# vghuy17ck1/svt-av1-psyex

Hardware: AMD Instinct MI355X
Metric: ME+RD-cost Mpixels/s (2160p10 preset-6) (higher is better)
Workload: dtype u8 SAD / i32 transforms; 1 GPU; 3840x2160 10-bit synthetic pan sequence, preset 6 (M6) search controls at qp 35; step = 16 pictures (4 current pictures x ref distance 1,2,4,8; R=2): open-loop ME of all 2040 b64 + full-pel pred + RD chain (64x64,32x32,16x16 DCT_DCT, 10-bit, b quantizer; qcoeff + recon + scalars written); 3 picture sets alternate from step to step

## Files before the change

### svt-av1-psyex_amd/csrc/rd_kernel.hip

```cpp
#include <hip/hip_runtime.h>
#include <math.h>
#include <stdint.h>
#include <string.h>
#include <type_traits>
#include "svt_hip_internal.h"
#include "../../include/svt_hip_dsp.h"

#include "txfm_core.h"

namespace {

struct RdParams {
    SvtHipRdBatchDesc d;
    const int16_t    *iscan[3];
    int               tx_size;
};

template <typename T> __device__ __forceinline__ int ldpix(const void *p, size_t i) { return (int)static_cast<const T *>(p)[i]; }

template <int LW> __device__ __forceinline__ u64 seg_sum_u64(u64 v) {
#pragma unroll
    for (int o = LW / 2; o > 0; o >>= 1) v += __shfl_xor(v, o, 64);
    return v;
}
template <int LW> __device__ __forceinline__ uint32_t seg_sum_u32(uint32_t v) {
#pragma unroll
    for (int o = LW / 2; o > 0; o >>= 1) v += __shfl_xor(v, o, 64);
    return v;
}
template <int LW> __device__ __forceinline__ uint32_t seg_max_u32(uint32_t v) {
#pragma unroll
    for (int o = LW / 2; o > 0; o >>= 1) { const uint32_t t = __shfl_xor(v, o, 64); v = t > v ? t : v; }
    return v;
}

__host__ __device__ constexpr int rd_lanes_per_block(int ts) { return tx_wide(ts) > tx_high(ts) ? tx_wide(ts) : tx_high(ts); }
__host__ __device__ constexpr int rd_blocks_per_wave(int ts) { return 64 / rd_lanes_per_block(ts); }

#ifndef SVT_RD_WAVES_64
#define SVT_RD_WAVES_64 2
#endif
#ifndef SVT_RD_WAVES_32
#define SVT_RD_WAVES_32 4
#endif
#ifndef SVT_RD_RESIDUAL_AHEAD
#define SVT_RD_RESIDUAL_AHEAD 8
#endif
#ifndef SVT_RD_SCAN_AHEAD
#define SVT_RD_SCAN_AHEAD 16
#endif
#ifndef SVT_RD_WAVES_16
#define SVT_RD_WAVES_16 4
#endif
__host__ __device__ constexpr int rd_waves_per_simd(int ts) {
    return rd_lanes_per_block(ts) == 64 ? SVT_RD_WAVES_64 : rd_lanes_per_block(ts) == 32 ? SVT_RD_WAVES_32 : SVT_RD_WAVES_16;
}
template <int TS, int BD> __global__ void __launch_bounds__(64, rd_waves_per_simd(TS)) rd_tx_kernel(const RdParams p) {
    constexpr int W = tx_wide(TS), H = tx_high(TS), WP = W > 32 ? 32 : W, HP = H > 32 ? 32 : H, NP = WP * HP;
    constexpr int LW = rd_lanes_per_block(TS), BPW = rd_blocks_per_wave(TS);
    constexpr bool kShift32 = LW != 32;
    constexpr int PA = W + 1, PB = WP + 1;
    constexpr int ROW_CLAMP = BD == 8 ? 16 : 18, COL_CLAMP = 16;
    constexpr bool RECT = (W == 2 * H || H == 2 * W);
    using Pix = typename std::conditional<BD == 8, uint8_t, uint16_t>::type;
    __shared__ int32_t lds[BPW][H * PA];
    const int      lane = threadIdx.x, blk = lane / LW, l = lane % LW;
    const uint32_t job   = blockIdx.x * BPW + blk;
    const bool     valid = job < p.d.n_jobs;
    int32_t *A = lds[blk];
    const SvtHipTxJob jb = p.d.jobs[valid ? job : 0];
    const int tt = jb.tx_type & 15, vt = c_vtx[tt], ht = c_htx[tt];
    const bool ud = (vt == 2), lr = (ht == 2);
    const Pix *src  = static_cast<const Pix *>(p.d.src) + jb.src_offset;
    const Pix *pred = static_cast<const Pix *>(p.d.pred) + jb.pred_offset;
    const int8_t *fsh = c_fwd_shift[TS];
    const int bit_col = c_fwd_cos_col[ilog2c(W) - 2][ilog2c(H) - 2], bit_row = c_fwd_cos_row[ilog2c(W) - 2][ilog2c(H) - 2];

    constexpr int RUN = W < 8 ? W : 8, RPR = W / RUN;
    typedef Pix __attribute__((ext_vector_type(RUN), aligned(sizeof(Pix)))) RunU;
    uint32_t rmax = 0;
    {
        HiLo rhl;
        constexpr int NIT = (RPR * H + LW - 1) / LW, kResidualAhead = NIT < SVT_RD_RESIDUAL_AHEAD ? NIT : SVT_RD_RESIDUAL_AHEAD;
        for (int it0 = 0; it0 < NIT; it0 += kResidualAhead) {
            RunU sv[kResidualAhead], pv[kResidualAhead];
#pragma unroll
            for (int j = 0; j < kResidualAhead; j++) {
                const int i = l + (it0 + j) * LW;
                if (it0 + j < NIT && i < RPR * H) {
                    const int r = i / RPR, c = (i - r * RPR) * RUN;
                    sv[j] = *reinterpret_cast<const RunU *>(src + (size_t)r * p.d.src_stride + c);
                    pv[j] = *reinterpret_cast<const RunU *>(pred + (size_t)r * p.d.pred_stride + c);
                }
            }
#pragma unroll
            for (int j = 0; j < kResidualAhead; j++) {
                const int i = l + (it0 + j) * LW;
                if (it0 + j < NIT && i < RPR * H) {
                    const int r = i / RPR, c = (i - r * RPR) * RUN;
#pragma unroll
                    for (int k = 0; k < RUN; k++) {
                        const int32_t d = (int16_t)((int16_t)sv[j][k] - (int16_t)pv[j][k]);
                        A[r * PA + c + k] = d;
                        rhl.take(d);
                    }
                }
            }
        }
        rmax = rhl.max_abs();
    }
    const bool fast_col = pass_fits_17_bits((uint32_t)__builtin_amdgcn_readfirstlane((int)seg_max_u32<64>(rmax)) << (fsh[0] > 0 ? fsh[0] : 0), H);
    __syncthreads();
    uint32_t cmax = 0;
    if (l < W) {
        int32_t x[H];
#pragma unroll
        for (int r = 0; r < H; r++) x[r] = A[(ud ? H - 1 - r : r) * PA + l];
        shift_vec<H>(x, fsh[0]);
        if (fast_col) { fwd_1d<H, 2>(x, vt, bit_col); shift_vec<H, kShift32>(x, fsh[1]); } else { fwd_1d<H, 0>(x, vt, bit_col); shift_vec<H>(x, fsh[1]); }
        const int oc = lr ? W - 1 - l : l;
#pragma unroll
        for (int r = 0; r < H; r++) A[r * PA + oc] = x[r];
        cmax = vec_max_abs<H>(x);
    }
    const bool fast_row = pass_fits_17_bits((uint32_t)__builtin_amdgcn_readfirstlane((int)seg_max_u32<64>(cmax)), W);
    __syncthreads();
    uint32_t comax = 0;
    if (l < H) {
        int32_t x[W];
#pragma unroll
        for (int c = 0; c < W; c++) x[c] = A[l * PA + c];
        if (fast_row) { fwd_1d<W, 2>(x, ht, bit_row); shift_vec<W, kShift32>(x, fsh[2]); } else { fwd_1d<W, 0>(x, ht, bit_row); shift_vec<W>(x, fsh[2]); }
        if constexpr (RECT) {
#pragma unroll
            for (int c = 0; c < W; c++) x[c] = rshift64((i64)x[c] * 5793, 12);
        }
#pragma unroll
        for (int c = 0; c < W; c++) A[l * PA + c] = x[c];
        comax = vec_max_abs<W>(x);
    }
    const bool q24 = (uint32_t)__builtin_amdgcn_readfirstlane((int)seg_max_u32<64>(comax)) < (1u << 16);
    __syncthreads();
    const int pf = jb.pf_shape & 3;
    const int keep_w = pf == 3 ? 1 : (W >> pf), keep_h = pf == 3 ? 1 : (H >> pf);
    u64 tq = 0;
    if (pf == 0) if constexpr (W > 32 || H > 32) {
        for (int i = l; i < W * H; i += LW) {
            const int r = i / W, c = i - r * W;
            if (r >= HP || c >= WP) { const int32_t v = A[r * PA + c]; tq += (u64)((i64)v * v); }
        }
        tq = seg_sum_u64<LW>(tq);
    }
    if constexpr (W > 32 || H > 32) __syncthreads();
    const SvtHipQuantRow q = p.d.quant_rows[jb.quant_row];
    const int     log_scale = p.d.quant_kind == 2 ? 0 : c_log_scale[TS];
    const int16_t *iscan    = p.iscan[(tt >= 10) ? ((tt & 1) ? 2 : 1) : 0];
    const uint8_t *qm = (tt < 9) ? p.d.qmatrix : nullptr, *iqm = (tt < 9) ? p.d.iqmatrix : nullptr;
    uint32_t satd = 0, eob = 0, qsum = 0;
    int32_t  dc_q = 0;
    u64      dres = 0, dpred = 0;
    int32_t *co_out = (p.d.coeff && valid) ? p.d.coeff + (size_t)job * NP : nullptr;
    int32_t *q_out  = (p.d.qcoeff && valid) ? p.d.qcoeff + (size_t)job * NP : nullptr;
    int32_t *dq_out = (p.d.dqcoeff && valid) ? p.d.dqcoeff + (size_t)job * NP : nullptr;
    const int32_t zb_c[2]  = {log_scale ? ((q.zbin[0] + (1 << (log_scale - 1))) >> log_scale) : q.zbin[0], log_scale ? ((q.zbin[1] + (1 << (log_scale - 1))) >> log_scale) : q.zbin[1]};
    const int32_t rnd_c[2] = {log_scale ? ((q.round[0] + (1 << (log_scale - 1))) >> log_scale) : q.round[0], log_scale ? ((q.round[1] + (1 << (log_scale - 1))) >> log_scale) : q.round[1]};
    const bool fast_q = q24 && !qm && p.d.quant_kind == 0 && !co_out && !dq_out && __all(pf == 0);
    if (fast_q) {
        static_assert(NP % LW == 0, "every lane of a block walks the same number of coefficients");
        constexpr int kScanAhead = NP / LW < SVT_RD_SCAN_AHEAD ? ((NP / LW) & ~1) : SVT_RD_SCAN_AHEAD;
        static_assert(kScanAhead >= 2 && kScanAhead % 2 == 0 && NP / LW >= kScanAhead, "ahead of the loop");
        uint32_t scan2[kScanAhead / 2];
#pragma unroll
        for (int k = 0; k < kScanAhead; k += 2) scan2[k / 2] = (uint32_t)(uint16_t)iscan[l + LW * k] | ((uint32_t)(uint16_t)iscan[l + LW * (k + 1)] << 16);
        auto one = [&](int rc, int32_t zb, int32_t rnd, int32_t quant, int32_t qshift, int32_t deq, int ahead = -1) {
            const int r = rc / WP, c = rc - r * WP;
            const int32_t co = A[r * PA + c], sign = co >> 31, a = (co ^ sign) - sign;
            satd += (uint32_t)a;
            int32_t t = a + rnd;
            if (BD == 8) t = t > 32767 ? 32767 : t;
            const int32_t tmp = mul24_shr(t, quant, 11) + (t << 5);
            int32_t qv = mul24_shr(tmp, qshift, 21 - log_scale);
            qv = a >= zb ? qv : 0;
            const int32_t dq = __mul24(qv, deq) >> log_scale;
            const int32_t qs = (qv ^ sign) - sign, dqs = (dq ^ sign) - sign;
            uint32_t e;
            if (ahead >= 0) e = qv ? ((scan2[ahead >> 1] >> (16 * (ahead & 1))) & 0xFFFFu) + 1u : 0u;
            else e = qv ? (uint32_t)iscan[rc] + 1u : 0u;
            eob = e > eob ? e : eob;
            qsum += (uint32_t)(qv > 63 ? 63 : qv);
            const int32_t dd = a - dq;
            dres += (u64)(uint32_t)__mul24(dd, dd);
            dpred += (u64)(uint32_t)__umul24((uint32_t)a, (uint32_t)a);
            A[r * PB + c] = dqs;
            if (q_out) q_out[rc] = qs;
            return qs;
        };
        const int ac0 = l != 0;
        dc_q = one(l, zb_c[ac0], rnd_c[ac0], q.quant[ac0], q.quant_shift[ac0], q.dequant[ac0], 0);
        const int32_t zb1 = zb_c[1], rnd1 = rnd_c[1], quant1 = q.quant[1], qshift1 = q.quant_shift[1], deq1 = q.dequant[1];
#pragma unroll
        for (int k = 1; k < kScanAhead; k++) one(l + LW * k, zb1, rnd1, quant1, qshift1, deq1, k);
        if constexpr (LW >= 32) {
            static_assert((NP / LW - kScanAhead) % 2 == 0, "pairs");
            for (int rc = l + kScanAhead * LW; rc < NP; rc += 2 * LW) {
                one(rc, zb1, rnd1, quant1, qshift1, deq1);
                one(rc + LW, zb1, rnd1, quant1, qshift1, deq1);
            }
        } else {
#pragma unroll 4
            for (int rc = l + kScanAhead * LW; rc < NP; rc += LW) one(rc, zb1, rnd1, quant1, qshift1, deq1);
        }
    } else
    for (int rc = l; rc < NP; rc += LW) {
        const int r = rc / WP, c = rc - r * WP, ac = rc != 0;
        const bool kept = pf == 0 || (c < keep_w && r < keep_h);
        const int32_t co = kept ? A[r * PA + c] : 0, sign = co < 0 ? -1 : 0, a = (co ^ sign) - sign;
        satd += (uint32_t)a;
        int32_t qv = 0, dq = 0;
        const int32_t wt = qm ? qm[rc] : 32, iwt = qm ? iqm[rc] : 32;
        if (q24 && !qm) {
            if (p.d.quant_kind == 0) {
                if (a >= zb_c[ac]) {
                    int32_t t = a + rnd_c[ac];
                    if (BD == 8) t = t > 32767 ? 32767 : t;
                    const int32_t tmp = mul24_shr(t, q.quant[ac], 11) + (t << 5);
                    qv = mul24_shr(tmp, q.quant_shift[ac], 21 - log_scale);
                    dq = __mul24(qv, (int32_t)q.dequant[ac]) >> log_scale;
                }
            } else {
                const bool keep = (a << (1 + log_scale)) >= q.dequant[ac];
                if (keep) {
                    int32_t t = a + (log_scale ? ((q.round_fp[ac] + (1 << (log_scale - 1))) >> log_scale) : q.round_fp[ac]);
                    if (BD == 8) t = t < -32768 ? -32768 : (t > 32767 ? 32767 : t);
                    qv = mul24_shr(t, q.quant_fp[ac], 16 - log_scale);
                    dq = __mul24(qv, (int32_t)q.dequant[ac]) >> log_scale;
                }
            }
        } else if (p.d.quant_kind == 0 && !qm) {
            const int32_t zb = zb_c[ac];
            if (a >= zb) {
                int32_t t = a + rnd_c[ac];
                if (BD == 8) t = t > 32767 ? 32767 : t;
                const int32_t tw  = t << 5;
                const int32_t tmp = (int32_t)(((i64)tw * q.quant[ac]) >> 16) + tw;
                qv = (int32_t)(((i64)tmp * q.quant_shift[ac]) >> (16 - log_scale + 5));
                dq = (qv * (int32_t)q.dequant[ac]) >> log_scale;
            }
        } else if (p.d.quant_kind == 0) {
            const int32_t zb = log_scale ? ((q.zbin[ac] + (1 << (log_scale - 1))) >> log_scale) : q.zbin[ac];
            if ((i64)a * wt >= ((i64)zb << 5)) {
                i64 t = (i64)a + (log_scale ? ((q.round[ac] + (1 << (log_scale - 1))) >> log_scale) : q.round[ac]);
                if (BD == 8) t = t < -32768 ? -32768 : (t > 32767 ? 32767 : t);
                t *= wt;
                qv = (int32_t)(((((t * q.quant[ac]) >> 16) + t) * q.quant_shift[ac]) >> (16 - log_scale + 5));
                const int32_t deq = ((int32_t)q.dequant[ac] * iwt + 16) >> 5;
                dq = (qv * deq) >> log_scale;
            }
        } else if (!qm) {
            const bool keep = (BD == 8) ? (((i64)a << (1 + log_scale)) >= (int32_t)q.dequant[ac]) : ((a << (1 + log_scale)) >= q.dequant[ac]);
            if (keep) {
                i64 t = (i64)a + (log_scale ? ((q.round_fp[ac] + (1 << (log_scale - 1))) >> log_scale) : q.round_fp[ac]);
                if (BD == 8) t = t < -32768 ? -32768 : (t > 32767 ? 32767 : t);
                qv = (int32_t)((t * q.quant_fp[ac]) >> (16 - log_scale));
                dq = (qv * (int32_t)q.dequant[ac]) >> log_scale;
            }
        } else {
            if ((i64)a * wt >= ((int32_t)q.dequant[ac] << (5 - (1 + log_scale)))) {
                i64 t = (i64)a + (log_scale ? ((q.round_fp[ac] + (1 << (log_scale - 1))) >> log_scale) : q.round_fp[ac]);
                if (BD == 8) t = t < -32768 ? -32768 : (t > 32767 ? 32767 : t);
                qv = (int32_t)((t * q.quant_fp[ac] * wt) >> (16 - log_scale + 5));
                const int32_t deq = ((int32_t)q.dequant[ac] * iwt + 16) >> 5;
                dq = (qv * deq) >> log_scale;
            }
        }
        const int32_t qs = (qv ^ sign) - sign, dqs = (dq ^ sign) - sign;
        if (qv) { const uint32_t e = (uint32_t)iscan[rc] + 1; eob = e > eob ? e : eob; }
        qsum += (uint32_t)(qv > 63 ? 63 : qv);
        if (rc == 0) dc_q = qs;
        const i64 dd = (i64)co - dqs;
        dres += (u64)(dd * dd);
        dpred += (u64)((i64)co * co);
        A[r * PB + c] = dqs;
        if (co_out) co_out[rc] = co;
        if (q_out) q_out[rc] = qs;
        if (dq_out) dq_out[rc] = dqs;
    }
    satd  = seg_sum_u32<LW>(satd);
    qsum  = seg_sum_u32<LW>(qsum);
    eob   = seg_max_u32<LW>(eob);
    dres  = seg_sum_u64<LW>(dres);
    dpred = seg_sum_u64<LW>(dpred);
    __syncthreads();
    int32_t xr[W];
    uint32_t irmax = 0;
    if (l < H) {
#pragma unroll
        for (int c = 0; c < W; c++) {
            int32_t v = (l < HP && c < WP) ? A[l * PB + c] : 0;
            if constexpr (RECT) v = rshift64((i64)v * 2896, 12);
            xr[c] = clampv(v, BD + 8);
        }
        irmax = vec_max_abs<W>(xr);
    }
    const bool fast_irow = ipass_fits_18_bits((uint32_t)__builtin_amdgcn_readfirstlane((int)seg_max_u32<64>(irmax)), W);
    uint32_t icmax = 0;
    if (l < H) {
        if (fast_irow) inv_1d<W, ROW_CLAMP, 2>(xr, ht); else inv_1d<W, ROW_CLAMP, 1>(xr, ht);
        shift_vec<W, kShift32>(xr, c_inv_shift0[TS]);
#pragma unroll
        for (int c = 0; c < W; c++) A[l * PA + c] = xr[c];
        icmax = vec_max_abs<W>(xr);
    }
    const bool fast_icol = ipass_fits_18_bits((uint32_t)__builtin_amdgcn_readfirstlane((int)seg_max_u32<64>(icmax)), H);
    __syncthreads();
    u64 sse = 0;
    if (l < W) {
        int32_t x[H];
        const int ic = lr ? W - 1 - l : l;
#pragma unroll
        for (int r = 0; r < H; r++) x[r] = (r < HP) ? clampv(A[r * PA + ic], BD + 6 > 16 ? BD + 6 : 16) : 0;
        if (fast_icol) inv_1d<H, COL_CLAMP, 2>(x, vt); else inv_1d<H, COL_CLAMP, 1>(x, vt);
        shift_vec<H, kShift32>(x, -4);
#pragma unroll
        for (int r = 0; r < H; r++) A[r * PA + l] = x[ud ? H - 1 - r : r];
    }
    __syncthreads();
    {
        Pix *rec = (p.d.recon && valid) ? static_cast<Pix *>(p.d.recon) + jb.pred_offset : nullptr;
        constexpr int NIT = (RPR * H + LW - 1) / LW;
        RunU pv[NIT], sv[NIT];
#pragma unroll
        for (int it = 0; it < NIT; it++) {
            const int i = l + it * LW;
            if (i < RPR * H) {
                const int r = i / RPR, c = (i - r * RPR) * RUN;
                pv[it] = *reinterpret_cast<const RunU *>(pred + (size_t)r * p.d.pred_stride + c);
                sv[it] = *reinterpret_cast<const RunU *>(src + (size_t)r * p.d.src_stride + c);
            }
        }
#pragma unroll
        for (int it = 0; it < NIT; it++) {
            const int i = l + it * LW;
            if (i < RPR * H) {
                const int r = i / RPR, c = (i - r * RPR) * RUN;
                RunU out;
#pragma unroll
                for (int k = 0; k < RUN; k++) {
                    int v = (int)pv[it][k] + A[r * PA + c + k];
                    v = v < 0 ? 0 : (v > (1 << BD) - 1 ? (1 << BD) - 1 : v);
                    out[k] = (Pix)v;
                    const int e = (int)sv[it][k] - v;
                    sse += (u64)((uint32_t)e * (uint32_t)e);
                }
                if (rec) *reinterpret_cast<RunU *>(rec + (size_t)r * p.d.pred_stride + c) = out;
            }
        }
    }
    sse = seg_sum_u64<LW>(sse);
    if (l == 0 && valid) {
        p.d.eob[job]  = (uint16_t)eob;
        p.d.satd[job] = satd;
        p.d.dist_coeff[2 * (size_t)job]     = dres;
        p.d.dist_coeff[2 * (size_t)job + 1] = dpred;
        p.d.three_quad_energy[job] = tq;
        p.d.sse[job]  = sse;
        if (p.d.cul_level) p.d.cul_level[job] = (uint8_t)((qsum > 63 ? 63 : qsum) | (dc_q < 0 ? 64 : 0)) + (uint8_t)(dc_q > 0 ? 128 : 0);
    }
}

struct InvParams {
    SvtHipInvTxBatchDesc d;
};
template <int TS, int BD, typename Pix> __global__ void __launch_bounds__(64, rd_waves_per_simd(TS)) inv_tx_kernel(const InvParams p) {
    constexpr int W = tx_wide(TS), H = tx_high(TS), WP = W > 32 ? 32 : W, HP = H > 32 ? 32 : H, NP = WP * HP;
    constexpr int LW = rd_lanes_per_block(TS), BPW = rd_blocks_per_wave(TS);
    constexpr bool kShift32 = LW != 32;
    constexpr int PA = W + 1, PB = WP + 1;
    constexpr int ROW_CLAMP = BD == 8 ? 16 : 18, COL_CLAMP = 16;
    constexpr bool RECT = (W == 2 * H || H == 2 * W);
    __shared__ int32_t lds[BPW][H * PA];
    const int      lane = threadIdx.x, blk = lane / LW, l = lane % LW;
    const uint32_t job   = blockIdx.x * BPW + blk;
    const bool     valid = job < p.d.n_jobs;
    int32_t *A = lds[blk];
    const SvtHipTxJob jb = p.d.jobs[valid ? job : 0];
    const int tt = jb.tx_type & 15, vt = c_vtx[tt], ht = c_htx[tt];
    const bool ud = (vt == 2), lr = (ht == 2);
    const Pix *pred = static_cast<const Pix *>(p.d.pred) + jb.pred_offset;
    const int32_t *dq = p.d.dqcoeff + (size_t)(valid ? job : 0) * NP;
    for (int rc = l; rc < NP; rc += LW) { const int r = rc / WP, c = rc - r * WP; A[r * PB + c] = dq[rc]; }
    __syncthreads();
    int32_t xr[W];
    uint32_t irmax = 0;
    if (l < H) {
#pragma unroll
        for (int c = 0; c < W; c++) {
            int32_t v = (l < HP && c < WP) ? A[l * PB + c] : 0;
            if constexpr (RECT) v = rshift64((i64)v * 2896, 12);
            xr[c] = clampv(v, BD + 8);
        }
        irmax = vec_max_abs<W>(xr);
    }
    const bool fast_irow = ipass_fits_18_bits((uint32_t)__builtin_amdgcn_readfirstlane((int)seg_max_u32<64>(irmax)), W);
    uint32_t icmax = 0;
    if (l < H) {
        if (fast_irow) inv_1d<W, ROW_CLAMP, 2>(xr, ht); else inv_1d<W, ROW_CLAMP, 1>(xr, ht);
        shift_vec<W, kShift32>(xr, c_inv_shift0[TS]);
#pragma unroll
        for (int c = 0; c < W; c++) A[l * PA + c] = xr[c];
        icmax = vec_max_abs<W>(xr);
    }
    const bool fast_icol = ipass_fits_18_bits((uint32_t)__builtin_amdgcn_readfirstlane((int)seg_max_u32<64>(icmax)), H);
    __syncthreads();
    if (l < W) {
        int32_t x[H];
        const int ic = lr ? W - 1 - l : l;
#pragma unroll
        for (int r = 0; r < H; r++) x[r] = (r < HP) ? clampv(A[r * PA + ic], BD + 6 > 16 ? BD + 6 : 16) : 0;
        if (fast_icol) inv_1d<H, COL_CLAMP, 2>(x, vt); else inv_1d<H, COL_CLAMP, 1>(x, vt);
        shift_vec<H, kShift32>(x, -4);
#pragma unroll
        for (int r = 0; r < H; r++) A[r * PA + l] = x[ud ? H - 1 - r : r];
    }
    __syncthreads();
    if (valid) {
        Pix *rec = static_cast<Pix *>(p.d.recon) + jb.src_offset;
        for (int i = l; i < W * H; i += LW) {
            const int r = i / W, c = i - r * W;
            int v = (int)pred[(size_t)r * p.d.pred_stride + c] + A[r * PA + c];
            v = v < 0 ? 0 : (v > (1 << BD) - 1 ? (1 << BD) - 1 : v);
            rec[(size_t)r * p.d.recon_stride + c] = (Pix)v;
        }
    }
}

template <int BD, typename Pix> int launch_inv(SvtHipContext *ctx, const InvParams &p) {
    const dim3 b(64);
#define CASE(S) case S: hipLaunchKernelGGL((inv_tx_kernel<S, BD, Pix>), dim3((p.d.n_jobs + rd_blocks_per_wave(S) - 1) / rd_blocks_per_wave(S)), b, 0, ctx->stream, p); break;
    switch (p.d.tx_size) {
        CASE(0) CASE(1) CASE(2) CASE(3) CASE(4) CASE(5) CASE(6) CASE(7) CASE(8) CASE(9) CASE(10) CASE(11) CASE(12) CASE(13) CASE(14) CASE(15) CASE(16) CASE(17) CASE(18)
    default: return svt_hip_fail(ctx, SVT_HIP_ERR_BAD_PARAM, "tx_size %d", p.d.tx_size);
    }
#undef CASE
    SVT_HIP_CHECK(ctx, hipGetLastError());
    return SVT_HIP_OK;
}

struct FwdParams {
    SvtHipFwdTxBatchDesc d;
};
template <int TS> __global__ void __launch_bounds__(64, rd_waves_per_simd(TS)) fwd_tx_kernel(const FwdParams p) {
    constexpr int W = tx_wide(TS), H = tx_high(TS);
    constexpr int LW = rd_lanes_per_block(TS), BPW = rd_blocks_per_wave(TS);
    constexpr int PA = W + 1;
    constexpr bool RECT = (W == 2 * H || H == 2 * W);
    __shared__ int32_t lds[BPW][H * PA];
    const int      lane = threadIdx.x, blk = lane / LW, l = lane % LW;
    const uint32_t job   = blockIdx.x * BPW + blk;
    const bool     valid = job < p.d.n_jobs;
    int32_t *A = lds[blk];
    const SvtHipTxJob jb = p.d.jobs[valid ? job : 0];
    const int tt = jb.tx_type & 15, vt = c_vtx[tt], ht = c_htx[tt];
    const bool ud = (vt == 2), lr = (ht == 2);
    const int16_t *res = p.d.residual + jb.src_offset;
    const int8_t *fsh = c_fwd_shift[TS];
    const int bit_col = c_fwd_cos_col[ilog2c(W) - 2][ilog2c(H) - 2], bit_row = c_fwd_cos_row[ilog2c(W) - 2][ilog2c(H) - 2];
    uint32_t rmax = 0;
    for (int i = l; i < W * H; i += LW) {
        const int r = i / W, c = i - r * W;
        const int32_t d = res[(size_t)r * p.d.residual_stride + c];
        A[r * PA + c] = d;
        rmax = max(rmax, (uint32_t)(d < 0 ? -d : d));
    }
    const bool fast_col = pass_fits_17_bits((uint32_t)__builtin_amdgcn_readfirstlane((int)seg_max_u32<64>(rmax)) << (fsh[0] > 0 ? fsh[0] : 0), H);
    __syncthreads();
    uint32_t cmax = 0;
    if (l < W) {
        int32_t x[H];
#pragma unroll
        for (int r = 0; r < H; r++) x[r] = A[(ud ? H - 1 - r : r) * PA + l];
        shift_vec<H>(x, fsh[0]);
        if (fast_col) fwd_1d<H, 2>(x, vt, bit_col); else fwd_1d<H, 0>(x, vt, bit_col);
        shift_vec<H>(x, fsh[1]);
        const int oc = lr ? W - 1 - l : l;
#pragma unroll
        for (int r = 0; r < H; r++) { A[r * PA + oc] = x[r]; cmax = max(cmax, (uint32_t)(x[r] < 0 ? -x[r] : x[r])); }
    }
    const bool fast_row = pass_fits_17_bits((uint32_t)__builtin_amdgcn_readfirstlane((int)seg_max_u32<64>(cmax)), W);
    __syncthreads();
    if (l < H) {
        int32_t x[W];
#pragma unroll
        for (int c = 0; c < W; c++) x[c] = A[l * PA + c];
        if (fast_row) fwd_1d<W, 2>(x, ht, bit_row); else fwd_1d<W, 0>(x, ht, bit_row);
        shift_vec<W>(x, fsh[2]);
        if constexpr (RECT) {
#pragma unroll
            for (int c = 0; c < W; c++) x[c] = rshift64((i64)x[c] * 5793, 12);
        }
#pragma unroll
        for (int c = 0; c < W; c++) A[l * PA + c] = x[c];
    }
    __syncthreads();
    if (valid) {
        const int pf = jb.pf_shape & 3;
        const int keep_w = pf == 3 ? 1 : (W >> pf), keep_h = pf == 3 ? 1 : (H >> pf);
        int32_t *out = p.d.coeff + (size_t)job * W * H;
        for (int i = l; i < W * H; i += LW) { const int r = i / W, c = i - r * W; out[i] = (c < keep_w && r < keep_h) ? A[r * PA + c] : 0; }
    }
}

int launch_fwd(SvtHipContext *ctx, const FwdParams &p) {
    const dim3 b(64);
#define CASE(S) case S: hipLaunchKernelGGL((fwd_tx_kernel<S>), dim3((p.d.n_jobs + rd_blocks_per_wave(S) - 1) / rd_blocks_per_wave(S)), b, 0, ctx->stream, p); break;
    switch (p.d.tx_size) {
        CASE(0) CASE(1) CASE(2) CASE(3) CASE(4) CASE(5) CASE(6) CASE(7) CASE(8) CASE(9) CASE(10) CASE(11) CASE(12) CASE(13) CASE(14) CASE(15) CASE(16) CASE(17) CASE(18)
    default: return svt_hip_fail(ctx, SVT_HIP_ERR_BAD_PARAM, "tx_size %d", p.d.tx_size);
    }
#undef CASE
    SVT_HIP_CHECK(ctx, hipGetLastError());
    return SVT_HIP_OK;
}

template <int BD> int launch_size(SvtHipContext *ctx, const RdParams &p) {
    const dim3 b(64);
#define CASE(S) case S: hipLaunchKernelGGL((rd_tx_kernel<S, BD>), dim3((p.d.n_jobs + rd_blocks_per_wave(S) - 1) / rd_blocks_per_wave(S)), b, 0, ctx->stream, p); break;
    switch (p.tx_size) {
        CASE(0) CASE(1) CASE(2) CASE(3) CASE(4) CASE(5) CASE(6) CASE(7) CASE(8) CASE(9) CASE(10) CASE(11) CASE(12) CASE(13) CASE(14) CASE(15) CASE(16) CASE(17) CASE(18)
    default: return svt_hip_fail(ctx, SVT_HIP_ERR_BAD_PARAM, "tx_size %d", p.tx_size);
    }
#undef CASE
    SVT_HIP_CHECK(ctx, hipGetLastError());
    return SVT_HIP_OK;
}

int scan_order(int tx_size, int tx_type, int16_t *scan, int16_t *iscan) {
    const int w = tx_wide(tx_size) > 32 ? 32 : tx_wide(tx_size), h = tx_high(tx_size) > 32 ? 32 : tx_high(tx_size), n = w * h;
    int k = 0;
    if (tx_type >= 10 && (tx_type & 1) == 0) { for (int i = 0; i < n; i++) scan[k++] = (int16_t)i; }
    else if (tx_type >= 11) { for (int c = 0; c < w; c++) for (int r = 0; r < h; r++) scan[k++] = (int16_t)(r * w + c); }
    else
        for (int d = 0; d < w + h - 1; d++) {
            const int down = (w < h) ? 1 : (w > h) ? 0 : (d & 1);
            for (int i = 0; i <= d; i++) { const int r = down ? i : d - i, c = d - r; if (r < h && c < w) scan[k++] = (int16_t)(r * w + c); }
        }
    for (int i = 0; i < n; i++) iscan[scan[i]] = (int16_t)i;
    return n;
}

}

extern "C" {

int svt_hip_tx_size_wide(int tx_size) { return (tx_size >= 0 && tx_size < 19) ? tx_wide(tx_size) : 0; }
int svt_hip_tx_size_high(int tx_size) { return (tx_size >= 0 && tx_size < 19) ? tx_high(tx_size) : 0; }

int svt_hip_scan_order(int tx_size, int tx_type, int16_t *scan, int16_t *iscan) {
    if (tx_size < 0 || tx_size >= 19 || tx_type < 0 || tx_type >= 16 || !scan || !iscan) return 0;
    return scan_order(tx_size, tx_type, scan, iscan);
}

int svt_hip_rd_batch(SvtHipContext *ctx, const SvtHipRdBatchDesc *d) {
    if (!ctx || !d) return SVT_HIP_ERR_BAD_PARAM;
    if (d->n_jobs == 0) return SVT_HIP_OK;
    if ((d->bit_depth != 8 && d->bit_depth != 10) || d->quant_kind > 2)
        return svt_hip_fail(ctx, SVT_HIP_ERR_BAD_PARAM, "bit_depth %u / quant_kind %u", d->bit_depth, d->quant_kind);
    if (!d->src || !d->pred || !d->jobs || !d->quant_rows || !d->eob || !d->satd || !d->dist_coeff || !d->three_quad_energy || !d->sse)
        return svt_hip_fail(ctx, SVT_HIP_ERR_BAD_PARAM, "a mandatory pointer of the RD batch is null");
    if ((d->qmatrix == nullptr) != (d->iqmatrix == nullptr)) return svt_hip_fail(ctx, SVT_HIP_ERR_BAD_PARAM, "qmatrix and iqmatrix go together");
    hipSetDevice(ctx->device);
    RdParams p;
    p.d       = *d;
    p.tx_size = d->tx_size;
    if (p.tx_size < 0 || p.tx_size >= 19) return svt_hip_fail(ctx, SVT_HIP_ERR_BAD_PARAM, "tx_size %d", p.tx_size);
    for (int k = 0; k < 3; k++) p.iscan[k] = ctx->iscan_dev + ((size_t)p.tx_size * 3 + k) * 1024;
    return d->bit_depth == 8 ? launch_size<8>(ctx, p) : launch_size<10>(ctx, p);
}

}

namespace {
template <typename Pix> __device__ __forceinline__ void fullpel_pred_b64(const Pix *ref, uint32_t ref_stride, int width, int height, const uint32_t *sb_best_mv,
                                                                         int list, int ref_idx, uint32_t w64, int bx, int by, Pix *pred, uint32_t pred_stride,
                                                                         int vec_ok) {
    typedef Pix __attribute__((ext_vector_type(8), aligned(sizeof(Pix)))) RunU;
    typedef Pix __attribute__((ext_vector_type(8))) Run;
    const uint32_t b = (uint32_t)bx + (uint32_t)by * w64;
    const uint32_t *mvs = sb_best_mv + ((size_t)b * 8 + list * 4 + ref_idx) * 85 + 5;
    for (int seg = threadIdx.x; seg < 64 * 8; seg += 256) {
        const int ly = seg >> 3, lx = (seg & 7) * 8, x = bx * 64 + lx, y = by * 64 + ly;
        if (x >= width || y >= height) continue;
        const int qx = lx >> 4, qy = ly >> 4;
        const uint32_t mv = mvs[(qx & 1) | ((qy & 1) << 1) | ((qx >> 1) << 2) | ((qy >> 1) << 3)];
        const int mvx = (int16_t)(mv & 0xFFFF), mvy = (int16_t)(mv >> 16);
        int sy = y + mvy;
        sy = sy < 0 ? 0 : (sy > height - 1 ? height - 1 : sy);
        const int sx = x + mvx;
        const Pix *srow = ref + (size_t)sy * ref_stride;
        Pix       *drow = pred + (size_t)y * pred_stride + x;
        if (vec_ok && sx >= 0 && sx + 8 <= width && x + 8 <= width) {
            *reinterpret_cast<Run *>(drow) = *reinterpret_cast<const RunU *>(srow + sx);
        } else {
            for (int i = 0; i < 8 && x + i < width; i++) {
                int cx = sx + i;
                cx = cx < 0 ? 0 : (cx > width - 1 ? width - 1 : cx);
                drow[i] = srow[cx];
            }
        }
    }
}

template <typename Pix> __global__ void __launch_bounds__(256) fullpel_pred_kernel(const Pix *ref, uint32_t ref_stride, int width, int height,
                                                                                   const uint32_t *sb_best_mv, int list, int ref_idx, uint32_t w64, int by64_first,
                                                                                   Pix *pred, uint32_t pred_stride, int vec_ok) {
    fullpel_pred_b64<Pix>(ref, ref_stride, width, height, sb_best_mv, list, ref_idx, w64, (int)blockIdx.x, by64_first + (int)blockIdx.y, pred, pred_stride, vec_ok);
}

struct PredBatch {
    SvtHipPredJob job[SVT_HIP_PRED_MAX_JOBS];
};
template <typename Pix> __global__ void __launch_bounds__(256) fullpel_pred_batch_kernel(const PredBatch pb, uint32_t ref_stride, int width, int height, uint32_t w64,
                                                                                         uint32_t pred_stride, int vec_ok) {
    const SvtHipPredJob &j = pb.job[blockIdx.z];
    if (blockIdx.y >= j.b64_row_count) return;
    fullpel_pred_b64<Pix>(static_cast<const Pix *>(j.ref), ref_stride, width, height, j.sb_best_mv, j.list, j.ref_idx, w64, (int)blockIdx.x,
                          (int)(j.b64_row_start + blockIdx.y), static_cast<Pix *>(j.pred), pred_stride, vec_ok);
}
}

extern "C" int svt_hip_fullpel_pred(SvtHipContext *ctx, const void *ref, uint32_t ref_stride, uint32_t width, uint32_t height, uint8_t bit_depth,
                                    const uint32_t *sb_best_mv, uint8_t list, uint8_t ref_idx, uint32_t b64_row_start, uint32_t b64_row_count, void *pred,
                                    uint32_t pred_stride) {
    if (!ctx || !ref || !sb_best_mv || !pred || list > 1 || ref_idx > 3 || (bit_depth != 8 && bit_depth != 10) || !width || !height)
        return svt_hip_fail(ctx, SVT_HIP_ERR_BAD_PARAM, "svt_hip_fullpel_pred: bad argument");
    hipSetDevice(ctx->device);
    const uint32_t w64 = (width + 63) / 64, h64 = (height + 63) / 64;
    if (b64_row_start >= h64) return svt_hip_fail(ctx, SVT_HIP_ERR_BAD_PARAM, "svt_hip_fullpel_pred: b64_row_start %u >= %u", b64_row_start, h64);
    if (b64_row_count == 0 || b64_row_start + b64_row_count > h64) b64_row_count = h64 - b64_row_start;
    const dim3 g(w64, b64_row_count), blk(256);
    const size_t bpp = bit_depth == 8 ? 1 : 2;
    const int vec_ok = ((reinterpret_cast<uintptr_t>(pred) % (8 * bpp)) == 0 && pred_stride % 8 == 0) ? 1 : 0;
    if (bit_depth == 8)
        hipLaunchKernelGGL(fullpel_pred_kernel<uint8_t>, g, blk, 0, ctx->stream, static_cast<const uint8_t *>(ref), ref_stride, (int)width, (int)height,
                           sb_best_mv, (int)list, (int)ref_idx, w64, (int)b64_row_start, static_cast<uint8_t *>(pred), pred_stride, vec_ok);
    else
        hipLaunchKernelGGL(fullpel_pred_kernel<uint16_t>, g, blk, 0, ctx->stream, static_cast<const uint16_t *>(ref), ref_stride, (int)width, (int)height,
                           sb_best_mv, (int)list, (int)ref_idx, w64, (int)b64_row_start, static_cast<uint16_t *>(pred), pred_stride, vec_ok);
    SVT_HIP_CHECK(ctx, hipGetLastError());
    return SVT_HIP_OK;
}

extern "C" int svt_hip_fullpel_pred_batch(SvtHipContext *ctx, uint32_t ref_stride, uint32_t width, uint32_t height, uint8_t bit_depth, uint32_t pred_stride,
                                          uint32_t n_jobs, const SvtHipPredJob *jobs) {
    if (!ctx) return SVT_HIP_ERR_BAD_PARAM;
    if (!jobs || n_jobs == 0 || n_jobs > SVT_HIP_PRED_MAX_JOBS || (bit_depth != 8 && bit_depth != 10) || !width || !height)
        return svt_hip_fail(ctx, SVT_HIP_ERR_BAD_PARAM, "svt_hip_fullpel_pred_batch: bad argument (1..%d jobs)", SVT_HIP_PRED_MAX_JOBS);
    const uint32_t w64 = (width + 63) / 64, h64 = (height + 63) / 64;
    const size_t   bpp = bit_depth == 8 ? 1 : 2;
    PredBatch pb;
    memset(&pb, 0, sizeof(pb));
    uint32_t rows_max = 0;
    int      vec_ok   = pred_stride % 8 == 0;
    for (uint32_t i = 0; i < n_jobs; i++) {
        SvtHipPredJob j = jobs[i];
        if (!j.ref || !j.sb_best_mv || !j.pred || j.list > 1 || j.ref_idx > 3 || j.b64_row_start >= h64)
            return svt_hip_fail(ctx, SVT_HIP_ERR_BAD_PARAM, "svt_hip_fullpel_pred_batch: job %u: null pointer, list / ref_idx or b64_row_start %u out of range", i,
                                j.b64_row_start);
        if (j.b64_row_count == 0 || j.b64_row_start + j.b64_row_count > h64) j.b64_row_count = h64 - j.b64_row_start;
        rows_max = j.b64_row_count > rows_max ? j.b64_row_count : rows_max;
        vec_ok   = vec_ok && (reinterpret_cast<uintptr_t>(j.pred) % (8 * bpp)) == 0;
        pb.job[i] = j;
    }
    hipSetDevice(ctx->device);
    const dim3 g(w64, rows_max, n_jobs), blk(256);
    if (bit_depth == 8) hipLaunchKernelGGL(fullpel_pred_batch_kernel<uint8_t>, g, blk, 0, ctx->stream, pb, ref_stride, (int)width, (int)height, w64, pred_stride, vec_ok);
    else hipLaunchKernelGGL(fullpel_pred_batch_kernel<uint16_t>, g, blk, 0, ctx->stream, pb, ref_stride, (int)width, (int)height, w64, pred_stride, vec_ok);
    SVT_HIP_CHECK(ctx, hipGetLastError());
    return SVT_HIP_OK;
}

extern "C" int svt_hip_inv_txfm_batch(SvtHipContext *ctx, const SvtHipInvTxBatchDesc *d) {
    if (!ctx || !d) return SVT_HIP_ERR_BAD_PARAM;
    if (d->n_jobs == 0) return SVT_HIP_OK;
    if ((d->bit_depth != 8 && d->bit_depth != 10) || (d->sample_bytes != 1 && d->sample_bytes != 2) || (d->bit_depth == 10 && d->sample_bytes != 2))
        return svt_hip_fail(ctx, SVT_HIP_ERR_BAD_PARAM, "inverse batch: bit_depth %u with %u-byte samples", d->bit_depth, d->sample_bytes);
    if (d->tx_size >= SVT_HIP_TX_SIZES_ALL) return svt_hip_fail(ctx, SVT_HIP_ERR_BAD_PARAM, "tx_size %u", d->tx_size);
    if (!d->pred || !d->recon || !d->jobs || !d->dqcoeff) return svt_hip_fail(ctx, SVT_HIP_ERR_BAD_PARAM, "a pointer of the inverse batch is null");
    hipSetDevice(ctx->device);
    InvParams p;
    p.d = *d;
    if (d->bit_depth == 10) return launch_inv<10, uint16_t>(ctx, p);
    return d->sample_bytes == 1 ? launch_inv<8, uint8_t>(ctx, p) : launch_inv<8, uint16_t>(ctx, p);
}

extern "C" int svt_hip_fwd_txfm_batch(SvtHipContext *ctx, const SvtHipFwdTxBatchDesc *d) {
    if (!ctx || !d) return SVT_HIP_ERR_BAD_PARAM;
    if (d->n_jobs == 0) return SVT_HIP_OK;
    if (d->tx_size >= SVT_HIP_TX_SIZES_ALL) return svt_hip_fail(ctx, SVT_HIP_ERR_BAD_PARAM, "tx_size %u", d->tx_size);
    if (!d->residual || !d->jobs || !d->coeff) return svt_hip_fail(ctx, SVT_HIP_ERR_BAD_PARAM, "a pointer of the forward batch is null");
    hipSetDevice(ctx->device);
    FwdParams p;
    p.d = *d;
    return launch_fwd(ctx, p);
}

int svt_hip_rd_tables_init(SvtHipContext *ctx) {
    int32_t cosp[4][64];
    for (int b = 0; b < 4; b++)
        for (int j = 0; j < 64; j++) cosp[b][j] = (int32_t)(cos(3.14159265358979323846 * j / 128.0) * (double)(1 << (10 + b)) + 0.5);
    SVT_HIP_CHECK(ctx, hipMemcpyToSymbol(HIP_SYMBOL(c_cospi), cosp, sizeof(cosp)));
    const size_t bytes = sizeof(int16_t) * 19 * 3 * 1024;
    int16_t *tab = static_cast<int16_t *>(calloc(1, bytes)), scan[1024];
    if (!tab) return svt_hip_fail(ctx, SVT_HIP_ERR_NO_MEMORY, "iscan tables");
    for (int s = 0; s < 19; s++)
        for (int kind = 0; kind < 3; kind++) scan_order(s, kind == 0 ? 0 : (kind == 1 ? 10 : 11), scan, tab + ((size_t)s * 3 + kind) * 1024);
    int rc = SVT_HIP_OK;
    if (hipMalloc(reinterpret_cast<void **>(&ctx->iscan_dev), bytes) != hipSuccess) rc = svt_hip_fail(ctx, SVT_HIP_ERR_NO_MEMORY, "iscan tables");
    else if (hipMemcpy(ctx->iscan_dev, tab, bytes, hipMemcpyHostToDevice) != hipSuccess) rc = svt_hip_fail(ctx, SVT_HIP_ERR_LAUNCH, "iscan tables: copy failed");
    free(tab);
    return rc;
}

void svt_hip_rd_tables_free(SvtHipContext *ctx) {
    if (ctx->iscan_dev) hipFree(ctx->iscan_dev);
    ctx->iscan_dev = nullptr;
}
```

Measured before the change: 40270 Mpixels/s.

## Split wide RD transforms across two waves with half-butterfly per wave

For transform sizes that use a full 64-lane block and are at least 32 wide, the RD kernel now launches 128 threads per job. Each wave computes one half of every 1-D DCT: the even half and the odd half of the butterfly, or half the identity outputs. Cross-wave maxima and partial sums are exchanged through shared memory, and the coefficients are repacked to the narrower pitch before quantisation. The aim is to cut per-thread register pressure and serial work on the long 64/32-point transforms, at the cost of extra block-wide barriers and shared-memory traffic.

```diff
diff --git a/svt-av1-psyex_amd/csrc/rd_kernel.hip b/svt-av1-psyex_amd/csrc/rd_kernel.hip
--- a/svt-av1-psyex_amd/csrc/rd_kernel.hip
+++ b/svt-av1-psyex_amd/csrc/rd_kernel.hip
@@ -55,19 +55,152 @@
 __host__ __device__ constexpr int rd_waves_per_simd(int ts) {
     return rd_lanes_per_block(ts) == 64 ? SVT_RD_WAVES_64 : rd_lanes_per_block(ts) == 32 ? SVT_RD_WAVES_32 : SVT_RD_WAVES_16;
 }
-template <int TS, int BD> __global__ void __launch_bounds__(64, rd_waves_per_simd(TS)) rd_tx_kernel(const RdParams p) {
+
+__host__ __device__ constexpr bool rd_two_waves(int ts) { return rd_lanes_per_block(ts) == 64 && tx_wide(ts) >= 32; }
+__host__ __device__ constexpr int rd_tx_lanes(int ts) { return rd_two_waves(ts) ? 128 : rd_lanes_per_block(ts); }
+__host__ __device__ constexpr int rd_tx_blocks(int ts) { return rd_two_waves(ts) ? 1 : rd_blocks_per_wave(ts); }
+__host__ __device__ constexpr int rd_tx_threads(int ts) { return rd_two_waves(ts) ? 128 : 64; }
+__host__ __device__ constexpr int rd_tx_waves_per_simd(int ts) { return rd_two_waves(ts) ? 4 : rd_waves_per_simd(ts); }
+
+template <int N, typename F> __device__ __forceinline__ void for_own(int h, int type, F f) {
+    constexpr int M = N / 2;
+    if (type == 0 || N >= 32) {
+#pragma unroll
+        for (int k = 0; k < M; k++) f(k, k + h * M);
+    } else if (h == 0) {
+#pragma unroll
+        for (int k = 0; k < N; k++) f(k, k);
+    }
+}
+template <int N> __device__ __forceinline__ void identity_half(int32_t *x) {
+    int32_t t[N];
+#pragma unroll
+    for (int i = 0; i < N / 2; i++) t[i] = x[i];
+    identity<N>(t);
+#pragma unroll
+    for (int i = 0; i < N / 2; i++) x[i] = t[i];
+}
+template <int N, int FM, typename Ld> __device__ __forceinline__ void fwd_half(int32_t *x, int h, int type, int bit, int sh_in, int sh_out, Ld ld) {
+    constexpr int M = N / 2;
+    constexpr bool S32 = FM == 2;
+    const int32_t *c = c_cospi[bit - 10];
+    auto up = [&](int32_t v) { return (int32_t)((uint32_t)v << sh_in); };
+    if (type == 0) {
+#pragma unroll
+        for (int i = 0; i < M; i++) { const int32_t a = up(ld(i)), b = up(ld(N - 1 - i)); x[i] = h ? wsub(a, b) : wadd(a, b); }
+        if (h == 0) {
+            fdct_core<M, FM>(x, c, bit);
+            permute_brev<M>(x);
+        } else {
+            int32_t y[N];
+#pragma unroll
+            for (int i = 0; i < M; i++) y[N - 1 - i] = x[i];
+            OddFwd<M, 1, FM>::run(y, c, bit);
+            odd_final<M, false, FM>(y, c, bit);
+            permute_brev<M>(y + M);
+#pragma unroll
+            for (int i = 0; i < M; i++) x[i] = y[M + i];
+        }
+        shift_vec<M, S32>(x, sh_out);
+    } else if constexpr (N >= 32) {
+#pragma unroll
+        for (int i = 0; i < M; i++) x[i] = up(ld(i + h * M));
+        if (type == 3) identity_half<N>(x);
+        shift_vec<M, S32>(x, sh_out);
+    } else if (h == 0) {
+#pragma unroll
+        for (int i = 0; i < N; i++) x[i] = up(ld(i));
+        if (type == 3) identity<N>(x);
+        else fadst<N, FM>(x, c, bit);
+        shift_vec<N, S32>(x, sh_out);
+    }
+}
+template <int N, typename St> __device__ __forceinline__ void fwd_store(const int32_t *x, int h, int type, St st) {
+    constexpr int M = N / 2;
+    if (type == 0) {
+#pragma unroll
+        for (int j = 0; j < M; j++) st(2 * j + h, x[j]);
+    } else if constexpr (N >= 32) {
+#pragma unroll
+        for (int k = 0; k < M; k++) st(k + h * M, x[k]);
+    } else if (h == 0) {
+#pragma unroll
+        for (int k = 0; k < N; k++) st(k, x[k]);
+    }
+}
+template <int N, typename Ld> __device__ __forceinline__ void inv_load(int32_t *x, int h, int type, Ld ld) {
+    constexpr int M = N / 2;
+    if (type == 0) {
+        if (h == 0) {
+#pragma unroll
+            for (int j = 0; j < M; j++) x[j] = ld(2 * j);
+            permute_brev<M>(x);
+        } else {
+#pragma unroll
+            for (int j = 0; j < M; j++) x[j] = ld(2 * brevc(j, ilog2c(M)) + 1);
+        }
+    } else if constexpr (N >= 32) {
+#pragma unroll
+        for (int k = 0; k < M; k++) x[k] = ld(k + h * M);
+    } else if (h == 0) {
+#pragma unroll
+        for (int i = 0; i < N; i++) x[i] = ld(i);
+    }
+}
+template <int N, int CLAMP, int IM> __device__ __forceinline__ void inv_half(int32_t *x, int h, int type) {
+    constexpr int M = N / 2;
+    const int32_t *c = c_cospi[2];
+    if (type == 0) {
+        if (h == 0) idct_core<M, CLAMP, IM>(x, c, 12);
+        else {
+            int32_t y[N];
+#pragma unroll
+            for (int i = 0; i < M; i++) y[M + i] = x[i];
+            odd_final<M, true, IM>(y, c, 12);
+            OddInv<M, ilog2c(M) - 1, CLAMP, IM>::run(y, c, 12);
+#pragma unroll
+            for (int i = 0; i < M; i++) x[i] = y[M + i];
+        }
+    } else if constexpr (N >= 32) {
+        if (type == 3) identity_half<N>(x);
+    } else if (h == 0) {
+        if (type == 3) identity<N>(x);
+        else iadst<N, CLAMP, IM>(x, c, 12);
+    }
+}
+template <int N, int CLAMP, typename Ld> __device__ __forceinline__ void inv_meet(int32_t *x, int h, Ld ld) {
+    constexpr int M = N / 2;
+#pragma unroll
+    for (int k = 0; k < M; k++) {
+        const int32_t o = ld(N - 1 - k - h * M);
+        x[k] = clamp32(h ? o - x[k] : x[k] + o, CLAMP);
+    }
+}
+
+template <int TS, int BD> __global__ void __launch_bounds__(rd_tx_threads(TS), rd_tx_waves_per_simd(TS)) rd_tx_kernel(const RdParams p) {
     constexpr int W = tx_wide(TS), H = tx_high(TS), WP = W > 32 ? 32 : W, HP = H > 32 ? 32 : H, NP = WP * HP;
-    constexpr int LW = rd_lanes_per_block(TS), BPW = rd_blocks_per_wave(TS);
+    constexpr bool TWO = rd_two_waves(TS);
+    constexpr int LW = rd_tx_lanes(TS), BPW = rd_tx_blocks(TS);
+    constexpr int LR = LW > 64 ? 64 : LW;
     constexpr bool kShift32 = LW != 32;
     constexpr int PA = W + 1, PB = WP + 1;
     constexpr int ROW_CLAMP = BD == 8 ? 16 : 18, COL_CLAMP = 16;
     constexpr bool RECT = (W == 2 * H || H == 2 * W);
     using Pix = typename std::conditional<BD == 8, uint8_t, uint16_t>::type;
     __shared__ int32_t lds[BPW][H * PA];
+    __shared__ uint32_t xmax[5][2];
+    __shared__ u64      xsum[7];
     const int      lane = threadIdx.x, blk = lane / LW, l = lane % LW;
+    const int      wv = l >> 6, v = l & 63;
     const uint32_t job   = blockIdx.x * BPW + blk;
     const bool     valid = job < p.d.n_jobs;
     int32_t *A = lds[blk];
+    auto block_max = [&](uint32_t lane_max, int slot) {
+        const uint32_t m = (uint32_t)__builtin_amdgcn_readfirstlane((int)seg_max_u32<64>(lane_max));
+        if (v == 0) xmax[slot][wv] = m;
+        __syncthreads();
+        return xmax[slot][0] > xmax[slot][1] ? xmax[slot][0] : xmax[slot][1];
+    };
     const SvtHipTxJob jb = p.d.jobs[valid ? job : 0];
     const int tt = jb.tx_type & 15, vt = c_vtx[tt], ht = c_htx[tt];
     const bool ud = (vt == 2), lr = (ht == 2);
@@ -109,6 +242,45 @@
         }
         rmax = rhl.max_abs();
     }
+    bool q24;
+    if constexpr (TWO) {
+        const bool fast_col = pass_fits_17_bits(block_max(rmax, 0) << (fsh[0] > 0 ? fsh[0] : 0), H);
+        uint32_t cmax = 0;
+        {
+            int32_t x[H];
+            if (v < W) {
+                auto ld = [&](int r) { return A[(vt == 2 ? H - 1 - r : r) * PA + v]; };
+                if (fast_col) fwd_half<H, 2>(x, wv, vt, bit_col, fsh[0], fsh[1], ld); else fwd_half<H, 0>(x, wv, vt, bit_col, fsh[0], fsh[1], ld);
+            }
+            __syncthreads();
+            if (v < W) {
+                const int oc = lr ? W - 1 - v : v;
+                HiLo m;
+                fwd_store<H>(x, wv, vt, [&](int r, int32_t val) { A[r * PA + oc] = val; m.take(val); });
+                cmax = m.max_abs();
+            }
+        }
+        const bool fast_row = pass_fits_17_bits(block_max(cmax, 1), W);
+        uint32_t comax = 0;
+        {
+            int32_t x[W];
+            if (v < H) {
+                auto ld = [&](int c) { return A[v * PA + c]; };
+                if (fast_row) fwd_half<W, 2>(x, wv, ht, bit_row, 0, fsh[2], ld); else fwd_half<W, 0>(x, wv, ht, bit_row, 0, fsh[2], ld);
+            }
+            __syncthreads();
+            if (v < H) {
+                HiLo m;
+                fwd_store<W>(x, wv, ht, [&](int c, int32_t val) {
+                    if constexpr (RECT) val = rshift64((i64)val * 5793, 12);
+                    A[v * PA + c] = val;
+                    m.take(val);
+                });
+                comax = m.max_abs();
+            }
+        }
+        q24 = block_max(comax, 2) < (1u << 16);
+    } else {
     const bool fast_col = pass_fits_17_bits((uint32_t)__builtin_amdgcn_readfirstlane((int)seg_max_u32<64>(rmax)) << (fsh[0] > 0 ? fsh[0] : 0), H);
     __syncthreads();
     uint32_t cmax = 0;
@@ -139,8 +311,9 @@
         for (int c = 0; c < W; c++) A[l * PA + c] = x[c];
         comax = vec_max_abs<W>(x);
     }
-    const bool q24 = (uint32_t)__builtin_amdgcn_readfirstlane((int)seg_max_u32<64>(comax)) < (1u << 16);
-    __syncthreads();
+    q24 = (uint32_t)__builtin_amdgcn_readfirstlane((int)seg_max_u32<64>(comax)) < (1u << 16);
+    __syncthreads();
+    }
     const int pf = jb.pf_shape & 3;
     const int keep_w = pf == 3 ? 1 : (W >> pf), keep_h = pf == 3 ? 1 : (H >> pf);
     u64 tq = 0;
@@ -149,7 +322,16 @@
             const int r = i / W, c = i - r * W;
             if (r >= HP || c >= WP) { const int32_t v = A[r * PA + c]; tq += (u64)((i64)v * v); }
         }
-        tq = seg_sum_u64<LW>(tq);
+        tq = seg_sum_u64<LR>(tq);
+    }
+    constexpr int PQ = TWO ? PB : PA;
+    if constexpr (TWO) {
+        int32_t kept[NP / LW];
+#pragma unroll
+        for (int k = 0; k < NP / LW; k++) { const int rc = l + k * LW, r = rc / WP, c = rc - r * WP; kept[k] = A[r * PA + c]; }
+        __syncthreads();
+#pragma unroll
+        for (int k = 0; k < NP / LW; k++) { const int rc = l + k * LW, r = rc / WP, c = rc - r * WP; A[r * PB + c] = kept[k]; }
     }
     if constexpr (W > 32 || H > 32) __syncthreads();
     const SvtHipQuantRow q = p.d.quant_rows[jb.quant_row];
@@ -174,7 +356,7 @@
         for (int k = 0; k < kScanAhead; k += 2) scan2[k / 2] = (uint32_t)(uint16_t)iscan[l + LW * k] | ((uint32_t)(uint16_t)iscan[l + LW * (k + 1)] << 16);
         auto one = [&](int rc, int32_t zb, int32_t rnd, int32_t quant, int32_t qshift, int32_t deq, int ahead = -1) {
             const int r = rc / WP, c = rc - r * WP;
-            const int32_t co = A[r * PA + c], sign = co >> 31, a = (co ^ sign) - sign;
+            const int32_t co = A[r * PQ + c], sign = co >> 31, a = (co ^ sign) - sign;
             satd += (uint32_t)a;
             int32_t t = a + rnd;
             if (BD == 8) t = t > 32767 ? 32767 : t;
@@ -214,7 +396,7 @@
     for (int rc = l; rc < NP; rc += LW) {
         const int r = rc / WP, c = rc - r * WP, ac = rc != 0;
         const bool kept = pf == 0 || (c < keep_w && r < keep_h);
-        const int32_t co = kept ? A[r * PA + c] : 0, sign = co < 0 ? -1 : 0, a = (co ^ sign) - sign;
+        const int32_t co = kept ? A[r * PQ + c] : 0, sign = co < 0 ? -1 : 0, a = (co ^ sign) - sign;
         satd += (uint32_t)a;
         int32_t qv = 0, dq = 0;
         const int32_t wt = qm ? qm[rc] : 32, iwt = qm ? iqm[rc] : 32;
@@ -285,12 +467,65 @@
         if (q_out) q_out[rc] = qs;
         if (dq_out) dq_out[rc] = dqs;
     }
-    satd  = seg_sum_u32<LW>(satd);
-    qsum  = seg_sum_u32<LW>(qsum);
-    eob   = seg_max_u32<LW>(eob);
-    dres  = seg_sum_u64<LW>(dres);
-    dpred = seg_sum_u64<LW>(dpred);
-    __syncthreads();
+    satd  = seg_sum_u32<LR>(satd);
+    qsum  = seg_sum_u32<LR>(qsum);
+    eob   = seg_max_u32<LR>(eob);
+    dres  = seg_sum_u64<LR>(dres);
+    dpred = seg_sum_u64<LR>(dpred);
+    if constexpr (TWO) {
+        if (l == 64) { xsum[0] = satd; xsum[1] = qsum; xsum[2] = eob; xsum[3] = dres; xsum[4] = dpred; xsum[5] = tq; }
+    }
+    __syncthreads();
+    u64 sse = 0;
+    if constexpr (TWO) {
+        uint32_t icmax = 0;
+        {
+            int32_t x[W];
+            HiLo m;
+            if (v < H) inv_load<W>(x, wv, ht, [&](int c) {
+                int32_t val = (v < HP && c < WP) ? A[v * PB + c] : 0;
+                if constexpr (RECT) val = rshift64((i64)val * 2896, 12);
+                val = clampv(val, BD + 8);
+                m.take(val);
+                return val;
+            });
+            const bool fast_irow = ipass_fits_18_bits(block_max(m.max_abs(), 3), W);
+            if (v < H) {
+                if (fast_irow) inv_half<W, ROW_CLAMP, 2>(x, wv, ht); else inv_half<W, ROW_CLAMP, 1>(x, wv, ht);
+                if (ht == 0) for_own<W>(wv, 0, [&](int k, int c) { A[v * PA + c] = x[k]; });
+            }
+            __syncthreads();
+            if (v < H && ht == 0) inv_meet<W, ROW_CLAMP>(x, wv, [&](int c) { return A[v * PA + c]; });
+            __syncthreads();
+            if (v < H) {
+                HiLo mo;
+                for_own<W>(wv, ht, [&](int k, int c) {
+                    shift_vec<1, true>(&x[k], c_inv_shift0[TS]);
+                    A[v * PA + c] = x[k];
+                    mo.take(x[k]);
+                });
+                icmax = mo.max_abs();
+            }
+        }
+        const bool fast_icol = ipass_fits_18_bits(block_max(icmax, 4), H);
+        {
+            int32_t x[H];
+            const int ic = lr ? W - 1 - v : v;
+            if (v < W) inv_load<H>(x, wv, vt, [&](int r) { return (r < HP) ? clampv(A[r * PA + ic], BD + 6 > 16 ? BD + 6 : 16) : 0; });
+            __syncthreads();
+            if (v < W) {
+                if (fast_icol) inv_half<H, COL_CLAMP, 2>(x, wv, vt); else inv_half<H, COL_CLAMP, 1>(x, wv, vt);
+                if (vt == 0) for_own<H>(wv, 0, [&](int k, int r) { A[r * PA + v] = x[k]; });
+            }
+            __syncthreads();
+            if (v < W && vt == 0) inv_meet<H, COL_CLAMP>(x, wv, [&](int r) { return A[r * PA + v]; });
+            __syncthreads();
+            if (v < W) for_own<H>(wv, vt, [&](int k, int r) {
+                shift_vec<1, true>(&x[k], -4);
+                A[(vt == 2 ? H - 1 - r : r) * PA + v] = x[k];
+            });
+        }
+    } else {
     int32_t xr[W];
     uint32_t irmax = 0;
     if (l < H) {
@@ -313,7 +548,6 @@
     }
     const bool fast_icol = ipass_fits_18_bits((uint32_t)__builtin_amdgcn_readfirstlane((int)seg_max_u32<64>(icmax)), H);
     __syncthreads();
-    u64 sse = 0;
     if (l < W) {
         int32_t x[H];
         const int ic = lr ? W - 1 - l : l;
@@ -323,6 +557,7 @@
         shift_vec<H, kShift32>(x, -4);
 #pragma unroll
         for (int r = 0; r < H; r++) A[r * PA + l] = x[ud ? H - 1 - r : r];
+    }
     }
     __syncthreads();
     {
@@ -356,7 +591,20 @@
             }
         }
     }
-    sse = seg_sum_u64<LW>(sse);
+    sse = seg_sum_u64<LR>(sse);
+    if constexpr (TWO) {
+        if (l == 64) xsum[6] = sse;
+        __syncthreads();
+        if (l == 0) {
+            satd += (uint32_t)xsum[0];
+            qsum += (uint32_t)xsum[1];
+            eob = (uint32_t)xsum[2] > eob ? (uint32_t)xsum[2] : eob;
+            dres += xsum[3];
+            dpred += xsum[4];
+            tq += xsum[5];
+            sse += xsum[6];
+        }
+    }
     if (l == 0 && valid) {
         p.d.eob[job]  = (uint16_t)eob;
         p.d.satd[job] = satd;
@@ -523,8 +771,7 @@
 }
 
 template <int BD> int launch_size(SvtHipContext *ctx, const RdParams &p) {
-    const dim3 b(64);
-#define CASE(S) case S: hipLaunchKernelGGL((rd_tx_kernel<S, BD>), dim3((p.d.n_jobs + rd_blocks_per_wave(S) - 1) / rd_blocks_per_wave(S)), b, 0, ctx->stream, p); break;
+#define CASE(S) case S: hipLaunchKernelGGL((rd_tx_kernel<S, BD>), dim3((p.d.n_jobs + rd_tx_blocks(S) - 1) / rd_tx_blocks(S)), dim3(rd_tx_threads(S)), 0, ctx->stream, p); break;
     switch (p.tx_size) {
         CASE(0) CASE(1) CASE(2) CASE(3) CASE(4) CASE(5) CASE(6) CASE(7) CASE(8) CASE(9) CASE(10) CASE(11) CASE(12) CASE(13) CASE(14) CASE(15) CASE(16) CASE(17) CASE(18)
     default: return svt_hip_fail(ctx, SVT_HIP_ERR_BAD_PARAM, "tx_size %d", p.tx_size);
```

Result: no change. 40560 Mpixels/s, median of 6 (+0.7%).
